# drowe67/radae

Measured on AMD Instinct MI355X. Metric: vocoder-feature frames/sec (enc+chan+dec), model19, higher is better.
Workload: dtype f32 I/O, 2xf16 (22-bit) MFMA operands, f32 accumulate (refine: f64 MFMA)

## Files before the change

radae_amd/csrc/rade_rx.hip:

```cpp
#include "rade_devutil.h"
typedef unsigned u32x2 __attribute__((ext_vector_type(2)));

#define DQ_XB 96
#define DQ_HB 16
#define DQ_PEND_MAX 64
#ifndef DQ_GIS
#define DQ_GIS 292
#endif
__device__ __forceinline__ int dq_xoff(int t, int col) { return (t + 1) * (DQ_XB * 8) + ((((col >> 3) ^ (t & 15)) << 3) | (col & 7)); }
__device__ __forceinline__ int dq_hoff(int t, int col) { return t * (DQ_HB * 8) + ((((col >> 3) ^ (t & 15)) << 3) | (col & 7)); }
__device__ __forceinline__ void dq_split(float v, _Float16 &hi, _Float16 &lo) { const float x = 256.0f * v; hi = (_Float16)x; lo = (_Float16)(x - (float)hi); }

enum { DQ_OUT_X = 0, DQ_OUT_GI = 1, DQ_OUT_GLOBAL = 2 };
struct DqGemm {
    const unsigned short *wa; int nct;
    const float *bias; int N;
    const float *wscale;
    int from_hb;
    int ktap;
    int ks0, nks;
    int init_gi;
    int out, ocol, act;
    float *gout; int gstride;
};
// ... 160 lines not shown
            if (act == 2) {
                const f16x4 hh = *(const lds_f16x4 *)(hbh + dq_hoff(tt, n)), hl = *(const lds_f16x4 *)(hbl + dq_hoff(tt, n));
#pragma unroll
                for (int r = 0; r < 4; r++) v[r] = clamp1(((float)hh[r] + (float)hl[r]) * 0x1p-8f * gate_sigmoid(v[r]));
            } else {
#pragma unroll
                for (int r = 0; r < 4; r++) v[r] = clamp1(gate_tanh(v[r]));
            }
            f16x4 oh, ol;
#pragma unroll
            for (int r = 0; r < 4; r++) { _Float16 a, b; dq_split(v[r], a, b); oh[r] = a; ol[r] = b; }
            *(lds_f16x4 *)(xh + dq_xoff(tt, ocol + n)) = oh; *(lds_f16x4 *)(xl + dq_xoff(tt, ocol + n)) = ol;
        }
    }
}
template <int NT>
__device__ __forceinline__ void dq2_gemm_tiles(DecShared2 *sh, const DqGemm g, int ct, int Tb, unsigned rstmask, int sync_first)
{
    if (uni_ptr(g.wscale) != nullptr) dq2_gemm_tiles_<NT, true>(sh, g, ct, Tb, rstmask, sync_first);
    else dq2_gemm_tiles_<NT, false>(sh, g, ct, Tb, rstmask, sync_first);
}

__device__ void dq2_dense1(DecShared2 *sh, const float *z, const rd_lin w, int Tb)
{
    constexpr int NKB = RD_LATENT / 8;
    const int lane = threadIdx.x & 63, nt = threadIdx.x >> 6, half = lane >> 5;
    if (nt >= 3) return;
    const float *wp = w.wp + ((size_t)nt * 64 + lane) * 4;
    const size_t wstep = (size_t)3 * 256;
    const int col = nt * 32 + (lane & 31);
    const float bias = w.bias[col];
    const int t = min(lane & 31, Tb - 1);
    const float *p1 = z + (size_t)t * RD_LATENT + 4 * half;
    f32x4 av[NKB], bv[NKB];
#pragma unroll
    for (int kb = 0; kb < NKB; kb++) { av[kb] = *(const f32x4 *)(p1 + kb * 8); bv[kb] = *(const f32x4 *)(wp + kb * wstep); }
    f32x16 acc;
#pragma unroll
    for (int j = 0; j < 16; j++) acc[j] = 0.0f;
#pragma unroll
    for (int kb = 0; kb < NKB; kb++)
#pragma unroll
        for (int s = 0; s < 4; s++) acc = __builtin_amdgcn_mfma_f32_32x32x2f32(av[kb][s], bv[kb][s], acc, 0, 0, 0);
#pragma unroll
    for (int j = 0; j < 16; j++) {
        const int tt = (j & 3) + 8 * (j >> 2) + 4 * half;
        if (tt >= Tb) continue;
        _Float16 a, b; dq_split(clamp1(gate_tanh(acc[j] + bias)), a, b);
        sh->xh[0][dq_xoff(tt, col)] = a; sh->xl[0][dq_xoff(tt, col)] = b;
    }
}

__device__ __forceinline__ f32x2 fma2(f32x2 a, f32x2 b, f32x2 c) { return (f32x2){ fmaf(a[0], b[0], c[0]), fmaf(a[1], b[1], c[1]) }; }
__device__ void dq2_scan(DecShared2 *sh, const float *Whh, const float *bhh, float *hstate, int Tb, unsigned rstmask)
{
    constexpr int H = 96, KP = H / 2;
    const int tid = rx_tid();
    const bool on = tid < 2 * H;
    const int j = on ? tid >> 1 : 0, p = tid & 1;
    f32x2 wr[KP / 2], wz[KP / 2], wn[KP / 2];
    {
        const float *w0 = Whh + (size_t)j * H + p * KP;
#pragma unroll
        for (int k = 0; k < KP; k += 4) {
            const f32x4 v0 = *(const f32x4 *)(w0 + k), v1 = *(const f32x4 *)(w0 + (size_t)H * H + k), v2 = *(const f32x4 *)(w0 + (size_t)2 * H * H + k);
#pragma unroll
            for (int u = 0; u < 2; u++) {
                wr[k / 2 + u] = (f32x2){ v0[2 * u], v0[2 * u + 1] }; wz[k / 2 + u] = (f32x2){ v1[2 * u], v1[2 * u + 1] }; wn[k / 2 + u] = (f32x2){ v2[2 * u], v2[2 * u + 1] };
            }
        }
    }
    const float br = bhh[j], bz = bhh[H + j], bn = bhh[2 * H + j];
    float hj = hstate[j];
    __syncthreads();
    if (on && p == 0) sh->hs[0][j] = hj;
    const float *gi = &sh->gi[0][0] + j;
    float g0r = gi[0], g0z = gi[H], g0n = gi[2 * H];
    __syncthreads();
    int cur = 0;
    for (int t = 0; t < Tb; t++) {
        if ((rstmask >> t) & 1u) {
            hj = 0.0f;
            __syncthreads();
            if (on && p == 0) sh->hs[cur][j] = 0.0f;
            __syncthreads();
        }
        const float *gn_ = gi + (size_t)min(t + 1, Tb - 1) * DQ_GIS;
        const float g1r = gn_[0], g1z = gn_[H], g1n = gn_[2 * H];
        f32x2 ar = { 0.0f, 0.0f }, az = { 0.0f, 0.0f }, an = { 0.0f, 0.0f }, ar2 = { 0.0f, 0.0f }, az2 = { 0.0f, 0.0f }, an2 = { 0.0f, 0.0f };
        const float *hp = sh->hs[cur] + p * KP;
#pragma unroll
        for (int k = 0; k < KP; k += 8) {
            const f32x4 hv = *(const f32x4 *)(hp + k), hw = *(const f32x4 *)(hp + k + 4);
            const f32x2 h0 = { hv[0], hv[1] }, h1 = { hv[2], hv[3] }, h2 = { hw[0], hw[1] }, h3 = { hw[2], hw[3] };
            ar = fma2(wr[k / 2], h0, ar); az = fma2(wz[k / 2], h0, az); an = fma2(wn[k / 2], h0, an);
            ar2 = fma2(wr[k / 2 + 1], h1, ar2); az2 = fma2(wz[k / 2 + 1], h1, az2); an2 = fma2(wn[k / 2 + 1], h1, an2);
            ar = fma2(wr[k / 2 + 2], h2, ar); az = fma2(wz[k / 2 + 2], h2, az); an = fma2(wn[k / 2 + 2], h2, an);
            ar2 = fma2(wr[k / 2 + 3], h3, ar2); az2 = fma2(wz[k / 2 + 3], h3, az2); an2 = fma2(wn[k / 2 + 3], h3, an2);
        }
        ar += ar2; az += az2; an += an2;
        float sr = ar[0] + ar[1], sz = az[0] + az[1], sn = an[0] + an[1];
        sr += quad_dpp<QUAD_XOR1>(sr); sz += quad_dpp<QUAD_XOR1>(sz); sn += quad_dpp<QUAD_XOR1>(sn);
        const float r = gate_sigmoid((sr + br) + g0r);
        const float z = gate_sigmoid((sz + bz) + g0z);
        const float n = gate_tanh(g0n + (sn + bn) * r);
        hj = (hj - n) * z + n;
        if (on && p == 0) {
            sh->hs[cur ^ 1][j] = hj;
            _Float16 a, b; dq_split(clamp1(hj), a, b);
            sh->hbh[0][dq_hoff(t, j)] = a; sh->hbl[0][dq_hoff(t, j)] = b;
        }
        g0r = g1r; g0z = g1z; g0n = g1n;
        cur ^= 1;
        if (t + 1 < Tb) __syncthreads();
    }
    if (on && p == 0) hstate[j] = hj;
}

template <int NB>
__device__ __forceinline__ void dq2_scan_mfma_body(DecShared2 *sh, const unsigned short *whq, const float *whs, const float *bhh, float *hstate, int Tb, unsigned rstmask, int ub0)
{
    constexpr int H = 96;
    const int tid = rx_tid(), lane = tid & 63, c = lane & 15, g = lane >> 4, cs = c & 3, par = c & 1;
    const int blk = NB == 2 ? (c >> 3) & 1 : 0;
    typedef const __attribute__((address_space(1))) f16x8 glb_f16x8_t;
    f16x8 A[NB][3][3];
    float sc[3], bb[3];
    const bool finl = (c & 4) == 0 && (NB == 2 || c < 4);
    const int ju = 16 * (ub0 + blk) + 4 * g + cs;
#pragma unroll
    for (int k = 0; k < NB; k++)
#pragma unroll
        for (int gate = 0; gate < 3; gate++)
#pragma unroll
            for (int ks = 0; ks < 3; ks++) A[k][gate][ks] = *(glb_f16x8_t *)(whq + (((size_t)ks * 18 + gate * 6 + ub0 + k) * 64 + lane) * 8);
#pragma unroll
    for (int gate = 0; gate < 3; gate++) { sc[gate] = whs[gate * H + ju] * 0x1p-8f; bb[gate] = bhh[gate * H + ju]; }
    float hj = hstate[ju];
    __syncthreads();
    _Float16 (*hp)[2][H] = (_Float16 (*)[2][H])&sh->hs[0][0];
    if (finl) { _Float16 a, b; dq_split(hj, a, b); hp[0][0][ju] = a; hp[0][1][ju] = b; }
    const float *gi = &sh->gi[0][0];
    float g0[3];
#pragma unroll
    for (int gate = 0; gate < 3; gate++) g0[gate] = gi[gate * H + ju];
    __syncthreads();
    int cur = 0;
    for (int t = 0; t < Tb; t++) {
        if ((rstmask >> t) & 1u) {
            __syncthreads();
            hj = 0.0f; if (finl) { hp[cur][0][ju] = (_Float16)0.0f; hp[cur][1][ju] = (_Float16)0.0f; }
            __syncthreads();
        }
        const float *gn_ = gi + (size_t)min(t + 1, Tb - 1) * DQ_GIS;
        float g1[3];
#pragma unroll
        for (int gate = 0; gate < 3; gate++) g1[gate] = gn_[gate * H + ju];
        f16x8 bq[3];
#pragma unroll
        for (int ks = 0; ks < 3; ks++) bq[ks] = *(const f16x8 *)&hp[cur][par][32 * ks + 8 * g];
        __builtin_amdgcn_sched_barrier(0);
        f32x4 acc[NB][3];
#pragma unroll
        for (int k = 0; k < NB; k++)
#pragma unroll
            for (int gate = 0; gate < 3; gate++) acc[k][gate] = (f32x4){ 0.0f, 0.0f, 0.0f, 0.0f };
#pragma unroll
        for (int ks = 0; ks < 3; ks++)
#pragma unroll
            for (int k = 0; k < NB; k++)
#pragma unroll
                for (int gate = 0; gate < 3; gate++) acc[k][gate] = __builtin_amdgcn_mfma_f32_16x16x32_f16(A[k][gate][ks], bq[ks], acc[k][gate], 0, 0, 0);
        float s3[3];
#pragma unroll
        for (int gate = 0; gate < 3; gate++) {
            float sr[4];
#pragma unroll
            for (int r = 0; r < 4; r++) {
                const float v = NB == 2 ? (blk ? acc[NB - 1][gate][r] : acc[0][gate][r]) : acc[0][gate][r];
                sr[r] = v + quad_dpp<QUAD_XOR1>(v); asm volatile("" : "+v"(sr[r]));
            }
            const float s01 = (cs & 1) ? sr[1] : sr[0], s23 = (cs & 1) ? sr[3] : sr[2];
            s3[gate] = (cs & 2) ? s23 : s01;
        }
        {
            const float r = gate_sigmoid((s3[0] * sc[0] + bb[0]) + g0[0]);
            const float z = gate_sigmoid((s3[1] * sc[1] + bb[1]) + g0[1]);
            const float n = gate_tanh(g0[2] + (s3[2] * sc[2] + bb[2]) * r);
            hj = (hj - n) * z + n;
        }
        if (finl) {
            _Float16 a, b; dq_split(hj, a, b);
            hp[cur ^ 1][0][ju] = a; hp[cur ^ 1][1][ju] = b;
            dq_split(clamp1(hj), a, b);
            sh->hbh[0][dq_hoff(t, ju)] = a; sh->hbl[0][dq_hoff(t, ju)] = b;
        }
#pragma unroll
        for (int gate = 0; gate < 3; gate++) g0[gate] = g1[gate];
        cur ^= 1;
        if (t + 1 < Tb) __syncthreads();
    }
    if (finl) hstate[ju] = hj;
}
__device__ void dq2_scan_mfma(DecShared2 *sh, const unsigned short *whq, const float *whs, const float *bhh, float *hstate, int Tb, unsigned rstmask)
{
    const int wave = rx2_wave();
    if (wave < 2) dq2_scan_mfma_body<2>(sh, whq, whs, bhh, hstate, Tb, rstmask, 2 * wave);
    else dq2_scan_mfma_body<1>(sh, whq, whs, bhh, hstate, Tb, rstmask, 2 + wave);
}

__device__ void dq2_layers(DecShared2 *sh, const rd_decs_args &a, int b, const float *z, float *out, int Tb, unsigned rstmask, int census_noscan)
{
    const int tid = rx_tid(), wave = tid >> 6;
    PH2_T0();
    {
        const unsigned *hist = (const unsigned *)(a.x + (size_t)b * a.x_sb - RD_DEC_W);
        constexpr int NH_ = (RD_DEC_W + NT2 - 1) / NT2;
        unsigned hu[NH_];
#pragma unroll
        for (int q = 0; q < NH_; q++) hu[q] = hist[min(tid + q * NT2, RD_DEC_W - 1)];
#pragma unroll
        for (int q = 0; q < NH_; q++) {
            const int c = tid + q * NT2; const unsigned u = hu[q];
            if (c < RD_DEC_W) { sh->xh[0][dq_xoff(-1, c)] = __builtin_bit_cast(_Float16, (unsigned short)(u & 0xffffu)); sh->xl[0][dq_xoff(-1, c)] = __builtin_bit_cast(_Float16, (unsigned short)(u >> 16)); }
        }
        for (int c = tid; c < DQ_XB * 8; c += NT2) { sh->xh[DQ2_ROWS + 1][c] = (_Float16)0.0f; sh->xl[DQ2_ROWS + 1][c] = (_Float16)0.0f; }
    }
    dq2_dense1(sh, z, a.dense1, Tb);
    DqGemm g;
    const int ct18 = wave < 2 ? 5 * wave : 10 + 4 * (wave - 2);
    g = (DqGemm){ a.gin[0].wa16, 18, a.gin[0].bias, 288, a.gin[0].wscale, 0, 0, 0, 3, 0, DQ_OUT_GI, 0, 0, nullptr, 0 };
    if (wave < 2) dq2_gemm_tiles<5>(sh, g, ct18, Tb, rstmask, 1); else dq2_gemm_tiles<4>(sh, g, ct18, Tb, rstmask, 1);
    PH2(20);
#pragma unroll 1
    for (int l = 0; l < 5; l++) {
        const int in = 96 + 128 * l, cin = in + 96;
        if (census_noscan) __syncthreads();
        else if (a.whq[l]) dq2_scan_mfma(sh, a.whq[l], a.whs[l], a.bhh[l], a.h[l] + (size_t)b * 96, Tb, rstmask);
        else dq2_scan(sh, a.whh[l], a.bhh[l], a.h[l] + (size_t)b * 96, Tb, rstmask);
        PH2(21);
        g = (DqGemm){ a.glu[l].wa16, 6, nullptr, 96, a.glu[l].wscale, 1, 0, 0, 3, 0, DQ_OUT_X, in, 2, nullptr, 0 };
        if (wave < 2) dq2_gemm_tiles<2>(sh, g, 2 * wave, Tb, rstmask, 1); else dq2_gemm_tiles<1>(sh, g, 2 + wave, Tb, rstmask, 1);
        PH2(22);
        const DqGemm gc = (DqGemm){ a.conv[l].wa16, 2, a.conv[l].bias, 32, a.conv[l].wscale, 0, cin / 32, 0, 2 * cin / 32, 0, DQ_OUT_X, cin, 1, nullptr, 0 };
        const bool last = l == 4;
        const rd_lin &nx = last ? a.output : a.gin[l + 1];
        const int nct = last ? 6 : 18;
        const DqGemm gm = (DqGemm){ nx.wa16, nct, nx.bias, last ? a.out_w : 288, nx.wscale, 0, 0, 0, cin / 32, 0, DQ_OUT_GI, 0, 0, nullptr, 0 };
        if (wave < 2) {
            dq2_gemm_tiles<1>(sh, gc, wave, Tb, rstmask, 1);
            if (!last) dq2_gemm_tiles<3>(sh, gm, 3 * wave, Tb, rstmask, 0);
        } else if (last) dq2_gemm_tiles<3>(sh, gm, 3 * (wave - 2), Tb, rstmask, 1);
        else {
            dq2_gemm_tiles<3>(sh, gm, 6 + 6 * (wave - 2), Tb, rstmask, 1);
            dq2_gemm_tiles<3>(sh, gm, 9 + 6 * (wave - 2), Tb, rstmask, 0);
        }
        PH2(23);
        const DqGemm gf = (DqGemm){ nx.wa16, nct, nullptr, last ? a.out_w : 288, nx.wscale, 0, 0, cin / 32, 1, 1, last ? DQ_OUT_GLOBAL : DQ_OUT_GI, 0, 0, out, a.out_w };
        if (last) { if (wave >= 2) dq2_gemm_tiles<3>(sh, gf, 3 * (wave - 2), Tb, rstmask, 1); else __syncthreads(); }
        else if (wave < 2) dq2_gemm_tiles<5>(sh, gf, ct18, Tb, rstmask, 1);
        else dq2_gemm_tiles<4>(sh, gf, ct18, Tb, rstmask, 1);
        PH2(24);
    }
    __syncthreads();
    {
        unsigned *hist = (unsigned *)(a.x + (size_t)b * a.x_sb - RD_DEC_W);
        for (int c = tid; c < RD_DEC_W; c += NT2)
            hist[c] = (unsigned)__builtin_bit_cast(unsigned short, sh->xh[0][dq_xoff(Tb - 1, c)]) | ((unsigned)__builtin_bit_cast(unsigned short, sh->xl[0][dq_xoff(Tb - 1, c)]) << 16);
    }
    __syncthreads();
}

struct RxShared2 {
    RxScalars S;
    double2 rq[4], rzc, rph[24], rrot[24]; double ral[24];
    int rows48[48];
    double redd[(NW2 + 1) * 10];
    float redf[16]; int redi[16]; int redj[16];
    double corrp[NW2][8];
    union {
      struct {
        float2 rxb[RD_RXBUF];
        float rowsum1[RD_NMF], rowsum2[RD_NMF];
        union {
          struct {
            __attribute__((aligned(16))) float2 xm[1408];
            double2 pd[RD_M], pendd[RD_M];
            float2 sym[6][RD_NC]; float2 rp[2][RD_NC];
            float eqP[RD_NC]; float2 eqPmat[RD_NC][2][3], eqrot[RD_NC]; float eq_pg, eq_snrc1, eq_snrc2, eq_pad;
            float2 cisA[2][18], cisB[2][64];
            union {
              struct {
                u32x2 rxhl[RD_RXBUF];
                double rmom[2][2][64][4];
                double mtot[2][16][16];
              };
              struct {
                double2 rtw[80], rrot80[80], rt80[80];
                float2 dtr[2 * 80 * 16];
              };
            };
          };
          struct {
            __attribute__((aligned(16))) _Float16 sA[2][2 * 2 * 2 * 64 * 8];
            __attribute__((aligned(16))) _Float16 sA2[5 * 2 * 64 * 8];
            unsigned srxh[RD_RXBUF], srxl[RD_RXBUF];
          };
        };
      };
      __attribute__((aligned(16))) unsigned char dec_raw[sizeof(DecShared2)];
    };
};
static_assert(sizeof(RxShared2) <= 80 * 1024, "two k_rx_sync2 workgroups must fit the 160 KiB LDS of a CU");

__device__ void block_argmax2(RxShared2 *sh, float &v, int &k0, int &k1)
{
    const int tid = rx_tid(), lane = tid & 63, wave = tid >> 6;
#define ARGMAX_STEP(CTRL) do { const float ov = quad_dpp<CTRL>(v); const int o0 = quad_dpp_i<CTRL>(k0), o1 = quad_dpp_i<CTRL>(k1); \
        if (ov > v || (ov == v && (o0 < k0 || (o0 == k0 && o1 < k1)))) { v = ov; k0 = o0; k1 = o1; } } while (0)
    ARGMAX_STEP(QUAD_XOR1); ARGMAX_STEP(QUAD_XOR2); ARGMAX_STEP(ROW_ROR4); ARGMAX_STEP(ROW_ROR8);
#undef ARGMAX_STEP
    {
        float bv = __int_as_float(__builtin_amdgcn_readlane(__float_as_int(v), 0)); int b0 = __builtin_amdgcn_readlane(k0, 0), b1 = __builtin_amdgcn_readlane(k1, 0);
#pragma unroll
        for (int r = 1; r < 4; r++) {
            const float ov = __int_as_float(__builtin_amdgcn_readlane(__float_as_int(v), 16 * r)); const int o0 = __builtin_amdgcn_readlane(k0, 16 * r), o1 = __builtin_amdgcn_readlane(k1, 16 * r);
            if (ov > bv || (ov == bv && (o0 < b0 || (o0 == b0 && o1 < b1)))) { bv = ov; b0 = o0; b1 = o1; }
        }
        v = bv; k0 = b0; k1 = b1;
    }
    if (lane == 0) { sh->redf[1 + wave] = v; sh->redi[1 + wave] = k0; sh->redj[1 + wave] = k1; }
    __syncthreads();
    float bv = sh->redf[1]; int b0 = sh->redi[1], b1 = sh->redj[1];
#pragma unroll
    for (int w = 1; w < NW2; w++) {
        const float ov = sh->redf[1 + w]; const int o0 = sh->redi[1 + w], o1 = sh->redj[1 + w];
        if (ov > bv || (ov == bv && (o0 < b0 || (o0 == b0 && o1 < b1)))) { bv = ov; b0 = o0; b1 = o1; }
    }
    v = bv; k0 = b0; k1 = b1;
}
template <int NV>
__device__ void block_sum_multi2(RxShared2 *sh, double (&v)[NV])
{
    const int tid = rx_tid(), lane = tid & 63, wave = tid >> 6;
#pragma unroll
    for (int k = 0; k < NV; k++) v[k] = wave_sum_f64(v[k]);
    if (lane == 0) {
#pragma unroll
        for (int k = 0; k < NV; k++) sh->redd[wave * NV + k] = v[k];
    }
    __syncthreads();
#pragma unroll
    for (int k = 0; k < NV; k++) {
        double t = 0.0;
#pragma unroll
        for (int w = 0; w < NW2; w++) t += sh->redd[w * NV + k];
        v[k] = t;
    }
}
__device__ float sigma_r_from_rowsums2(RxShared2 *sh)
{
    double v[2] = { 0.0, 0.0 };
    for (int t = rx_tid(); t < RD_NMF; t += NT2) { v[0] += (double)sh->rowsum1[t]; v[1] += (double)sh->rowsum2[t]; }
    block_sum_multi2<2>(sh, v);
    return sigma_r_from_sums(v[0], v[1]);
}


struct MomPlanes { f16x8 h, m, l; };
__device__ __forceinline__ MomPlanes mom_split(const f32x4 a0, const f32x4 a1)
{
    MomPlanes p;
#pragma unroll
    for (int j = 0; j < 8; j++) {
        const float v = 0x1p-7f * (j < 4 ? a0[j & 3] : a1[j & 3]);
        const _Float16 h = (_Float16)v; const float r1 = v - (float)h;
        const _Float16 m = (_Float16)r1; const float r2 = r1 - (float)m;
        p.h[j] = h; p.m[j] = m; p.l[j] = (_Float16)r2;
    }
    return p;
}
__device__ __forceinline__ f32x4 mom_expand(const f16x8 ah, const f16x8 al, const MomPlanes &p)
{
    f32x4 c = { 0.0f, 0.0f, 0.0f, 0.0f };
    c = __builtin_amdgcn_mfma_f32_16x16x32_f16(ah, p.l, c, 0, 0, 0);
    c = __builtin_amdgcn_mfma_f32_16x16x32_f16(al, p.m, c, 0, 0, 0);
    c = __builtin_amdgcn_mfma_f32_16x16x32_f16(al, p.h, c, 0, 0, 0);
    c = __builtin_amdgcn_mfma_f32_16x16x32_f16(ah, p.m, c, 0, 0, 0);
    c = __builtin_amdgcn_mfma_f32_16x16x32_f16(ah, p.h, c, 0, 0, 0);
    return c;
}
__device__ __forceinline__ void rx2_detect_q(RxShared2 *sh, const unsigned short *corrq16_, const unsigned short *corra16_, float *cache_, int cached, int oldb, int newb,
                                             float rx_unsc_, float &best, int &bt, int &bfi)
{
    constexpr int RT = 5, NTF = 5, TPW = 15;
    static_assert(TPW * NW2 * 16 == RD_NMF && TPW % RT == 0, "timing tiles per wavefront");
    const int tid = rx_tid(), wave = rx2_wave(), lane = tid & 63, i = lane & 15, g = lane >> 4;
    const float rx_unsc = rx_unsc_ * 0x1p-3f;
    const __amdgpu_buffer_rsrc_t qrs = __builtin_amdgcn_make_buffer_rsrc((void *)uni_ptr(corrq16_), 0, 2 * 10 * 2048, 0x00020000);
    const int vo = tid * 16;
    u32x4 stg[2];
    auto stage_load = [&](int sb) {
        stg[0] = __builtin_amdgcn_raw_buffer_load_b128(qrs, vo, sb * 4096, 0); stg[1] = __builtin_amdgcn_raw_buffer_load_b128(qrs, vo, sb * 4096 + 10 * 2048, 0);
    };
    auto stage_store = [&](int buf) { _Float16 *d = &sh->sA[buf][tid * 8]; *(u32x4 *)d = stg[0]; *(u32x4 *)(d + 256 * 8) = stg[1]; };
    PH2_T0();
    {
        const __amdgpu_buffer_rsrc_t ars = __builtin_amdgcn_make_buffer_rsrc((void *)uni_ptr(corra16_), 0, 5 * 2048, 0x00020000);
        const u32x4 t0 = __builtin_amdgcn_raw_buffer_load_b128(ars, vo, 0, 0), t1 = __builtin_amdgcn_raw_buffer_load_b128(ars, vo, 4096, 0);
        u32x4 t2 = { 0u, 0u, 0u, 0u };
        if (wave < 2) t2 = __builtin_amdgcn_raw_buffer_load_b128(ars, vo, 8192, 0);
        stage_load(0);
        _Float16 *d = &sh->sA2[tid * 8];
        *(u32x4 *)d = t0; *(u32x4 *)(d + 256 * 8) = t1;
        if (wave < 2) *(u32x4 *)(d + 512 * 8) = t2;
        stage_store(0);
    }
    float lbest = best; int lkey = 0x7fffffff;
    int pb = 0;
    __syncthreads();
    PH2(15);
#pragma unroll 1
    for (int pass = cached ? 1 : 0; pass < 2; pass++) {
        const unsigned *ph = sh->srxh + pass * RD_NMF + i + 4 * g, *pl = sh->srxl + pass * RD_NMF + i + 4 * g;
        const __amdgpu_buffer_rsrc_t drs = __builtin_amdgcn_make_buffer_rsrc((void *)uni_ptr(cache_ + (size_t)(pass ? newb : oldb) * RD_NFC * RD_NMF), 0, RD_NFC * RD_NMF * 4, 0x00020000);
        const __amdgpu_buffer_rsrc_t prs = __builtin_amdgcn_make_buffer_rsrc((void *)uni_ptr(cache_ + (size_t)oldb * RD_NFC * RD_NMF), 0, RD_NFC * RD_NMF * 4, 0x00020000);
        float *rowsum = pass ? sh->rowsum2 : sh->rowsum1;
#pragma unroll 1
        for (int grp = 0; grp < TPW / RT; grp++) {
            const int T0 = wave * TPW + grp * RT;
            f32x4 acc1[RT][2];
#pragma unroll
            for (int rt = 0; rt < RT; rt++) { acc1[rt][0] = (f32x4){ 0.0f, 0.0f, 0.0f, 0.0f }; acc1[rt][1] = (f32x4){ 0.0f, 0.0f, 0.0f, 0.0f }; }
            u32x4 wh[RT + 1], wl[RT + 1];
#pragma unroll
            for (int rt = 0; rt < RT; rt++)
#pragma unroll
                for (int j = 0; j < 4; j++) { wh[rt][j] = ph[16 * (T0 + rt) + j]; wl[rt][j] = pl[16 * (T0 + rt) + j]; }
#pragma unroll
            for (int sb = 0; sb < 5; sb++) {
                stage_load(sb == 4 ? 0 : sb + 1);
#pragma unroll
                for (int ds = 0; ds < 2; ds++) {
                    const int sidx = 2 * sb + ds;
                    if (sidx < 9) {
#pragma unroll
                        for (int j = 0; j < 4; j++) { wh[(RT + sidx) % (RT + 1)][j] = ph[16 * (T0 + RT + sidx) + j]; wl[(RT + sidx) % (RT + 1)][j] = pl[16 * (T0 + RT + sidx) + j]; }
                    }
                    const _Float16 *Ab = &sh->sA[pb][lane * 8];
                    const f16x8 a0h = *(const f16x8 *)(Ab + ((0 * 2 + ds) * 2 + 0) * 512), a0l = *(const f16x8 *)(Ab + ((0 * 2 + ds) * 2 + 1) * 512);
                    const f16x8 a1h = *(const f16x8 *)(Ab + ((1 * 2 + ds) * 2 + 0) * 512), a1l = *(const f16x8 *)(Ab + ((1 * 2 + ds) * 2 + 1) * 512);
                    __builtin_amdgcn_sched_barrier(0);
#define WSL(rt) (((rt) + sidx) % (RT + 1))
#pragma unroll
                    for (int rt = 0; rt < RT; rt++) acc1[rt][0] = __builtin_amdgcn_mfma_f32_16x16x32_f16(a0l, __builtin_bit_cast(f16x8, wh[WSL(rt)]), acc1[rt][0], 0, 0, 0);
#pragma unroll
                    for (int rt = 0; rt < RT; rt++) acc1[rt][1] = __builtin_amdgcn_mfma_f32_16x16x32_f16(a1l, __builtin_bit_cast(f16x8, wh[WSL(rt)]), acc1[rt][1], 0, 0, 0);
#pragma unroll
                    for (int rt = 0; rt < RT; rt++) acc1[rt][0] = __builtin_amdgcn_mfma_f32_16x16x32_f16(a0h, __builtin_bit_cast(f16x8, wl[WSL(rt)]), acc1[rt][0], 0, 0, 0);
#pragma unroll
                    for (int rt = 0; rt < RT; rt++) acc1[rt][1] = __builtin_amdgcn_mfma_f32_16x16x32_f16(a1h, __builtin_bit_cast(f16x8, wl[WSL(rt)]), acc1[rt][1], 0, 0, 0);
#pragma unroll
                    for (int rt = 0; rt < RT; rt++) acc1[rt][0] = __builtin_amdgcn_mfma_f32_16x16x32_f16(a0h, __builtin_bit_cast(f16x8, wh[WSL(rt)]), acc1[rt][0], 0, 0, 0);
#pragma unroll
                    for (int rt = 0; rt < RT; rt++) acc1[rt][1] = __builtin_amdgcn_mfma_f32_16x16x32_f16(a1h, __builtin_bit_cast(f16x8, wh[WSL(rt)]), acc1[rt][1], 0, 0, 0);
#undef WSL
                    __builtin_amdgcn_sched_barrier(0);
                }
                stage_store(pb ^ 1);
                pb ^= 1;
                __syncthreads();
            }
            PH2(16);
            f16x8 A2h[NTF], A2l[NTF];
#pragma unroll
            for (int q = 0; q < NTF; q++) { A2h[q] = *(const f16x8 *)&sh->sA2[((q * 2) * 64 + lane) * 8]; A2l[q] = *(const f16x8 *)&sh->sA2[((q * 2 + 1) * 64 + lane) * 8]; }
            const int gb = (wave * (TPW / RT) + grp) * RT * 2560;
            float pv[2][2 * NTF];
            auto pv_load = [&](int slot, int rt) {
                const u32x4 v0 = __builtin_amdgcn_raw_buffer_load_b128(prs, lane * 16, gb + rt * 2560, 0), v1 = __builtin_amdgcn_raw_buffer_load_b128(prs, lane * 16, gb + rt * 2560 + 1024, 0);
                const u32x2 v2 = __builtin_amdgcn_raw_buffer_load_b64(prs, lane * 8, gb + rt * 2560 + 2048, 0);
#pragma unroll
                for (int k = 0; k < 4; k++) { pv[slot][k] = __uint_as_float(v0[k]); pv[slot][4 + k] = __uint_as_float(v1[k]); }
                pv[slot][8] = __uint_as_float(v2[0]); pv[slot][9] = __uint_as_float(v2[1]);
            };
            if (pass) pv_load(0, 0);
            const int tb = 16 * T0 + i;
#pragma unroll
            for (int rt = 0; rt < RT; rt++) {
                if (pass && rt + 1 < RT) pv_load((rt + 1) & 1, rt + 1);
                const MomPlanes mp = mom_split(acc1[rt][0], acc1[rt][1]);
                float dd[2 * NTF], rs = 0.0f;
#pragma unroll
                for (int q = 0; q < NTF; q++) {
                    const f32x4 c = mom_expand(A2h[q], A2l[q], mp);
                    const float d0 = rx_unsc * __builtin_amdgcn_sqrtf(fmaf(c[0], c[0], c[1] * c[1])), d1 = rx_unsc * __builtin_amdgcn_sqrtf(fmaf(c[2], c[2], c[3] * c[3]));
                    rs += d0; rs += d1;
                    dd[2 * q] = d0; dd[2 * q + 1] = d1;
                }
                {
                    const auto p16 = __builtin_amdgcn_permlane16_swap(__float_as_uint(rs), __float_as_uint(rs), false, false);
                    rs = __uint_as_float(p16[0]) + __uint_as_float(p16[1]);
                    const auto p32 = __builtin_amdgcn_permlane32_swap(__float_as_uint(rs), __float_as_uint(rs), false, false);
                    rs = __uint_as_float(p32[0]) + __uint_as_float(p32[1]);
                }
                __builtin_amdgcn_raw_buffer_store_b128((u32x4){ __float_as_uint(dd[0]), __float_as_uint(dd[1]), __float_as_uint(dd[2]), __float_as_uint(dd[3]) }, drs, lane * 16, gb + rt * 2560, 0);
                __builtin_amdgcn_raw_buffer_store_b128((u32x4){ __float_as_uint(dd[4]), __float_as_uint(dd[5]), __float_as_uint(dd[6]), __float_as_uint(dd[7]) }, drs, lane * 16, gb + rt * 2560 + 1024, 0);
                __builtin_amdgcn_raw_buffer_store_b64((u32x2){ __float_as_uint(dd[8]), __float_as_uint(dd[9]) }, drs, lane * 8, gb + rt * 2560 + 2048, 0);
                const int t = tb + 16 * rt;
                if (pass) {
#pragma unroll
                    for (int q = 0; q < NTF; q++) {
                        const int k0 = (t << 6) | (8 * q + 2 * g);
                        const float s0 = pv[rt & 1][2 * q] + dd[2 * q], s1 = pv[rt & 1][2 * q + 1] + dd[2 * q + 1];
                        const bool c0 = s0 > lbest; lbest = c0 ? s0 : lbest; lkey = c0 ? k0 : lkey;
                        const bool c1 = s1 > lbest; lbest = c1 ? s1 : lbest; lkey = c1 ? k0 + 1 : lkey;
                    }
                }
                if (g == 0) rowsum[t] = rs;
            }
            PH2(17);
        }
        __syncthreads();
        PH2(18);
    }
    best = lbest; bt = lkey >> 6; bfi = lkey & 63;
}

__device__ __forceinline__ f64x4 refine2_tile(const RxShared2 *sh, int mt, int frame, int s0, int ns, int nf, int nt, int lane)
{
    const int i = lane & 15, kk = lane >> 4, c = kk & 1, n0 = kk >> 1;
    const int row = 16 * mt + i, fi = row >> 1, cp = row & 1;
    const bool rv = fi < nf;
    const double2 z1 = sh->rtw[rv ? fi : 0];
    double2 cur = s0 ? sh->rt80[rv ? fi : 0] : make_double2(1.0, 0.0);
    if (n0) cur = make_double2(cur.x * z1.x - cur.y * z1.y, cur.x * z1.y + cur.y * z1.x);
    const double c2r = z1.x * z1.x - z1.y * z1.y, c2i = 2.0 * z1.x * z1.y;
    const double2 prv = make_double2(cur.x * c2r + cur.y * c2i, cur.y * c2r - cur.x * c2i);
    double xc = cp == c ? cur.x : (cp == 0 ? -cur.y : cur.y), xp = cp == c ? prv.x : (cp == 0 ? -prv.y : prv.y);
    if (!rv) { xc = 0.0; xp = 0.0; }
    const double k2 = 2.0 * c2r;
    const double *xw = (const double *)&sh->xm[0] + 4 * (frame * 176 + (i < nt ? i : 0) + 2 * s0 + n0) + 2 * c;
    const double2 *pp = &sh->pd[2 * s0 + n0];
    f64x4 acc0 = { 0.0, 0.0, 0.0, 0.0 }, acc1 = acc0;
    double2 pn[4]; double a1[4], a2[4];
#pragma unroll
    for (int u = 0; u < 4; u++) { pn[u] = pp[2 * u]; a1[u] = xw[8 * u]; a2[u] = xw[8 * u + 1]; }
#pragma unroll 1
    for (int s = 0; s < ns; s += 4) {
        double b[4];
#pragma unroll
        for (int u = 0; u < 4; u++) b[u] = pn[u].x * a1[u];
#pragma unroll
        for (int u = 0; u < 4; u++) b[u] = fma(pn[u].y, a2[u], b[u]);
        __builtin_amdgcn_sched_barrier(0);
        const int sn = s + 4 < ns ? s + 4 : s;
#pragma unroll
        for (int u = 0; u < 4; u++) { pn[u] = pp[2 * (sn + u)]; a1[u] = xw[8 * (sn + u)]; a2[u] = xw[8 * (sn + u) + 1]; }
        __builtin_amdgcn_sched_barrier(0);
        const double x1 = fma(k2, xc, -xp), x2 = fma(k2, x1, -xc), x3 = fma(k2, x2, -x1);
        acc0 = __builtin_amdgcn_mfma_f64_16x16x4f64(xc, b[0], acc0, 0, 0, 0);
        acc1 = __builtin_amdgcn_mfma_f64_16x16x4f64(x1, b[1], acc1, 0, 0, 0);
        acc0 = __builtin_amdgcn_mfma_f64_16x16x4f64(x2, b[2], acc0, 0, 0, 0);
        acc1 = __builtin_amdgcn_mfma_f64_16x16x4f64(x3, b[3], acc1, 0, 0, 0);
        xp = x3; xc = fma(k2, x3, -x2);
        __builtin_amdgcn_sched_barrier(0);
    }
    return acc0 + acc1;
}
__device__ __forceinline__ void refine2_tables(RxShared2 *sh, int k, double fstart, double fstop, double fstep)
{
    const int nf = (int)ceil((fstop - fstart) / fstep);
    const double delta = (fstart + fstep) - fstart;
    if (k < 0 || k >= 3 * nf) return;
    const int which = k / nf, fi = k - which * nf;
    const double w = 2.0 * PI_D * dgrid_nc(fstart, fi, delta) / 8000.0;
    const double arg = which == 0 ? -w : (which == 1 ? -w * RD_NMF : -w * 80.0);
    double sn, cs; sincos(arg, &sn, &cs);
    double2 *dstp = which == 0 ? sh->rtw : (which == 1 ? sh->rrot80 : sh->rt80);
    dstp[fi] = make_double2(cs, sn);
}
__device__ __forceinline__ void refine2_tables_sync(RxShared2 *sh, int k, double fstart, double fstop, double fstep)
{
    const int nf = (int)ceil((fstop - fstart) / fstep);
    const double delta = (fstart + fstep) - fstart;
    const double wc = 0.5 * (2.0 * PI_D * fstart / 8000.0 + 2.0 * PI_D * dgrid_nc(fstart, nf - 1, delta) / 8000.0);
    if (k < 0 || k > 52) return;
    const int kf = k < 24 ? k : k - 24;
    if (k < 48 && kf >= nf) return;
    const double w = 2.0 * PI_D * dgrid_nc(fstart, kf, delta) / 8000.0, dw = w - wc;
    const double arg = k < 24 ? -w * RD_NMF : (k < 48 ? -dw * 79.5 : (k < 52 ? -wc * 40.0 * (k - 48) : -wc));
    double sn, cs; sincos(arg, &sn, &cs);
    const double2 v = make_double2(cs, sn);
    if (k < 24) sh->rrot[k] = v;
    else if (k < 48) { sh->rph[kf] = v; sh->ral[kf] = dw * 80.0; }
    else if (k < 52) sh->rq[k - 48] = v;
    else sh->rzc = v;
}
__device__ __forceinline__ void refine2_moments(const RxShared2 *sh, const double *vmg, int frame, int q, int nt, int lane, f64x4 &acc0, f64x4 &acc1)
{
    const int i = lane & 15, kk = lane >> 4, c = kk & 1, n0 = kk >> 1;
    const int m = i >> 1, cp = i & 1, s0 = 20 * q;
    const double2 z1 = sh->rzc;
    double2 cur = sh->rq[q];
    if (n0) cur = make_double2(cur.x * z1.x - cur.y * z1.y, cur.x * z1.y + cur.y * z1.x);
    const double c2r = z1.x * z1.x - z1.y * z1.y, c2i = 2.0 * z1.x * z1.y;
    const double2 prv = make_double2(cur.x * c2r + cur.y * c2i, cur.y * c2r - cur.x * c2i);
    double xc = cp == c ? cur.x : (cp == 0 ? -cur.y : cur.y), xp = cp == c ? prv.x : (cp == 0 ? -prv.y : prv.y);
    const double k2 = 2.0 * c2r;
    const double *xw = (const double *)&sh->xm[0] + 4 * (frame * 176 + (i < nt ? i : 0) + 2 * s0 + n0) + 2 * c;
    const double2 *pp = &sh->pd[2 * s0 + n0];
    const __attribute__((address_space(1))) double *vp = (const __attribute__((address_space(1))) double *)vmg + m * RD_M + 2 * s0 + n0;
    double vall[20];
#pragma unroll
    for (int u = 0; u < 20; u++) vall[u] = vp[2 * u];
    double2 pn[4]; double a1[4], a2[4];
#pragma unroll
    for (int u = 0; u < 4; u++) { pn[u] = pp[2 * u]; a1[u] = xw[8 * u]; a2[u] = xw[8 * u + 1]; }
#pragma unroll
    for (int s = 0; s < 20; s += 4) {
        double b[4];
#pragma unroll
        for (int u = 0; u < 4; u++) b[u] = pn[u].x * a1[u];
#pragma unroll
        for (int u = 0; u < 4; u++) b[u] = fma(pn[u].y, a2[u], b[u]);
        __builtin_amdgcn_sched_barrier(0);
        const int sn = s + 4 < 20 ? s + 4 : s;
#pragma unroll
        for (int u = 0; u < 4; u++) { pn[u] = pp[2 * (sn + u)]; a1[u] = xw[8 * (sn + u)]; a2[u] = xw[8 * (sn + u) + 1]; }
        __builtin_amdgcn_sched_barrier(0);
        const double x1 = fma(k2, xc, -xp), x2 = fma(k2, x1, -xc), x3 = fma(k2, x2, -x1);
        acc0 = __builtin_amdgcn_mfma_f64_16x16x4f64(xc * vall[s], b[0], acc0, 0, 0, 0);
        acc1 = __builtin_amdgcn_mfma_f64_16x16x4f64(x1 * vall[s + 1], b[1], acc1, 0, 0, 0);
        acc0 = __builtin_amdgcn_mfma_f64_16x16x4f64(x2 * vall[s + 2], b[2], acc0, 0, 0, 0);
        acc1 = __builtin_amdgcn_mfma_f64_16x16x4f64(x3 * vall[s + 3], b[3], acc1, 0, 0, 0);
        xp = x3; xc = fma(k2, x3, -x2);
        __builtin_amdgcn_sched_barrier(0);
    }
}

__device__ void rx2_refine(RxShared2 *sh, const double *vmg, int *tmax, double *fmax, int t0, int nt, double fstart, double fstop, double fstep, bool in_sync)
{
    const int tid = rx_tid(), lane = tid & 63, wave = tid >> 6;
    const int nf = (int)ceil((fstop - fstart) / fstep);
    const double delta = (fstart + fstep) - fstart;
    const int ntasks = ((2 * nf + 15) >> 4) * 2;
    const int i = lane & 15, kk = lane >> 4;
    PH2_T0();
    if (!in_sync) refine2_tables(sh, tid, fstart, fstop, fstep);
    for (int j = tid; j < 2 * 176; j += NT2) {
        const int frame = j / 176, k = j - frame * 176;
        const float2 x = sh->rxb[min(t0 + frame * RD_NMF + k, RD_RXBUF - 1)];
        double *d = (double *)&sh->xm[0] + 4 * j;
        d[0] = (double)x.x; d[1] = (double)x.y; d[2] = (double)x.y; d[3] = -(double)x.x;
    }
    __syncthreads();
    PH2(27);
    float best = -1.0f; int bf = 0x7fffffff, bt = 0x7fffffff;
    if (in_sync) {
        {
            f64x4 a0 = { 0.0, 0.0, 0.0, 0.0 }, a1 = a0;
            refine2_moments(sh, vmg, wave & 1, 2 * (wave >> 1), nt, lane, a0, a1);
            refine2_moments(sh, vmg, wave & 1, 2 * (wave >> 1) + 1, nt, lane, a0, a1);
            const f64x4 part = a0 + a1;
#pragma unroll
            for (int r = 0; r < 4; r++) sh->rmom[wave >> 1][wave & 1][lane][r] = part[r];
        }
        __syncthreads();
        PH2(28);
        for (int o = tid; o < 2 * 64 * 4; o += NT2) {
            const int frame = o >> 8, l = (o >> 2) & 63, r = o & 3;
            sh->mtot[frame][(l >> 4) + 4 * r][l & 15] = sh->rmom[0][frame][l][r] + sh->rmom[1][frame][l][r];
        }
        __syncthreads();
        PH2(29);
        for (int o = tid; o < nf * 16; o += NT2) {
            const int fo = o >> 4, t = o & 15;
            if (t >= nt) continue;
            const double al = sh->ral[fo];
            const double2 ph = sh->rph[fo], rt = sh->rrot[fo];
            float2 d12[2];
#pragma unroll
            for (int frame = 0; frame < 2; frame++) {
                double re = 0.0, im = 0.0, cm = 1.0;
#pragma unroll
                for (int mq = 0; mq < 8; mq++) {
                    const double mr = sh->mtot[frame][2 * mq][t], mi = sh->mtot[frame][2 * mq + 1][t];
                    if ((mq & 3) == 0) { re = fma(cm, mr, re); im = fma(cm, mi, im); }
                    else if ((mq & 3) == 1) { re = fma(cm, mi, re); im = fma(-cm, mr, im); }
                    else if ((mq & 3) == 2) { re = fma(-cm, mr, re); im = fma(-cm, mi, im); }
                    else { re = fma(-cm, mi, re); im = fma(cm, mr, im); }
                    cm = cm * al * (1.0 / (double)(mq + 1));
                }
                double xr = re * ph.x - im * ph.y, xi = re * ph.y + im * ph.x;
                if (frame == 1) { const double tr = xr * rt.x - xi * rt.y; xi = xr * rt.y + xi * rt.x; xr = tr; }
                d12[frame] = make_float2((float)xr, (float)xi);
            }
            const float v = hypotf(d12[0].x + d12[1].x, d12[0].y + d12[1].y);
            if (v > best || (v == best && (fo < bf || (fo == bf && t < bt)))) { best = v; bf = fo; bt = t; }
        }
    } else {
        auto finish = [&](const f64x4 &acc, int mt, int frame) {
#pragma unroll
            for (int r = 0; r < 4; r++) {
                const double mine = acc[r], other = __shfl_xor(mine, 16);
                if ((kk & 1) == 0) {
                    const int fo = 8 * mt + (kk >> 1) + 2 * r;
                    double re = mine, im = other;
                    if (frame == 1 && fo < nf) {
                        const double2 rt = sh->rrot80[fo];
                        const double tr = re * rt.x - im * rt.y; im = re * rt.y + im * rt.x; re = tr;
                    }
                    if (fo < nf && i < nt) sh->dtr[(frame * nf + fo) * 16 + i] = make_float2((float)re, (float)im);
                }
            }
        };
        for (int task = wave; task < ntasks; task += NW2) finish(refine2_tile(sh, task >> 1, task & 1, 0, 80, nf, nt, lane), task >> 1, task & 1);
        __syncthreads();
        for (int task = tid; task < nf * nt; task += NT2) {
            const int fi = task / nt, ti = task - fi * nt;
            const float2 a = sh->dtr[fi * 16 + ti], b = sh->dtr[(nf + fi) * 16 + ti];
            const float v = hypotf(a.x + b.x, a.y + b.y);
            if (v > best || (v == best && (fi < bf || (fi == bf && ti < bt)))) { best = v; bf = fi; bt = ti; }
        }
    }
    PH2(30);
    block_argmax2(sh, best, bf, bt);
    PH2(31);
    if (best > 0.0f) { *tmax = t0 + bt; *fmax = dgrid_nc(fstart, bf, delta); }
}

__device__ __forceinline__ void rx2_load_rxbuf(RxShared2 *sh, const rd_rx_stream *st, int tid)
{
    constexpr int NB_ = (RD_RXBUF + NT2 - 1) / NT2, NR_ = (RD_NMF + NT2 - 1) / NT2;
    float2 v[NB_]; float r1[NR_], r2[NR_];
#pragma unroll
    for (int q = 0; q < NB_; q++) { const int i = min(tid + q * NT2, RD_RXBUF - 1); v[q] = make_float2(st->rx_buf[i][0], st->rx_buf[i][1]); }
#pragma unroll
    for (int q = 0; q < NR_; q++) { const int i = min(tid + q * NT2, RD_NMF - 1); r1[q] = st->rowsum1[i]; r2[q] = st->rowsum2[i]; }
#pragma unroll
    for (int q = 0; q < NB_; q++) { const int i = tid + q * NT2; if (i < RD_RXBUF) sh->rxb[i] = v[q]; }
#pragma unroll
    for (int q = 0; q < NR_; q++) { const int i = tid + q * NT2; if (i < RD_NMF) { sh->rowsum1[i] = r1[q]; sh->rowsum2[i] = r2[q]; } }
}

__device__ __forceinline__ void rx2_decode_pending(RxShared2 *sh, const rd_sync_args &a, int b)
{
    RxScalars *S = &sh->S;
    DecShared2 *ds = (DecShared2 *)&sh->dec_raw[0];
    rd_rx_round *rnd = a.round + b;
    rd_rx_stream *st = a.st + b;
    const int tid = rx_tid();
    const int Tb = S->n_rows;
    PH2_T0();
    for (int i = tid; i < RD_RXBUF; i += NT2) { st->rx_buf[i][0] = sh->rxb[i].x; st->rx_buf[i][1] = sh->rxb[i].y; }
    for (int i = tid; i < RD_NMF; i += NT2) { st->rowsum1[i] = sh->rowsum1[i]; st->rowsum2[i] = sh->rowsum2[i]; }
    __syncthreads();
    PH2(19);
    for (int i = tid; i < Tb; i += NT2) ds->rst[i] = rnd->row_reset[i];
    if (tid == 0) S->lds_sync = 0;
    __syncthreads();
    for (int c0 = 0; c0 < Tb; c0 += DQ2_ROWS) {
        const int n = min(DQ2_ROWS, Tb - c0);
        unsigned rstmask = 0u;
        for (int t = 0; t < n; t++) rstmask |= ds->rst[c0 + t] ? (1u << t) : 0u;
        if (!CENSUS(1)) dq2_layers(ds, a.dec, b, a.dec.z + (size_t)b * a.dec.z_sb + (size_t)c0 * RD_LATENT, a.dec.out + (size_t)b * a.dec.out_sb + (size_t)c0 * a.dec.out_w, n, rstmask, CENSUS(2));
    }
    const float *f84 = a.dec.out + (size_t)b * a.dec.out_sb;
    for (int r = tid; r < Tb; r += NT2) ds->err[r] = f84[r * 84 + 20] > 0.0f ? 1 : 0;
    float *out = a.features_out + (size_t)b * a.feat_stride + (size_t)S->out_base * RD_FEAT_MF;
    for (int i0 = tid; i0 < (Tb / 3) * RD_FEAT_MF; i0 += 4 * NT2) {
        float v[4];
#pragma unroll
        for (int q = 0; q < 4; q++) {
            const int i = min(i0 + q * NT2, (Tb / 3) * RD_FEAT_MF - 1), fr = i / 36, j = i - fr * 36;
            const int row = fr >> 2, sub = fr & 3;
            v[q] = f84[row * 84 + sub * 21 + min(j, 19)];
            if (j >= 20) v[q] = 0.0f;
        }
#pragma unroll
        for (int q = 0; q < 4; q++) { const int i = i0 + q * NT2; if (i < (Tb / 3) * RD_FEAT_MF) out[i] = v[q]; }
    }
    __syncthreads();
    if (a.trace) {
        for (int c = S->batch_call0 + tid; c < S->n_calls; c += NT2) {
            const int idx = rnd->call_trace_idx[c];
            if (idx >= a.trace_cap) continue;
            int e = 0;
            for (int r = rnd->call_row_lo[c]; r < rnd->call_row_hi[c]; r++) e += ds->err[r];
            a.trace[(size_t)b * a.trace_cap + idx].uw_errors += e;
        }
    }
    if (tid == 0) {
        int add = 0;
        for (int r = S->uw_from_row; r < Tb; r++) add += ds->err[r];
        S->uw_errors += add;
        S->out_base += Tb / 3; S->n_rows = 0; S->uw_from_row = 0; S->pending_valid = 0; S->batch_call0 = S->n_calls; S->need_decode = 0;
    }
    __syncthreads();
    PH2_RESTART();
    rx2_load_rxbuf(sh, st, tid);
    __syncthreads();
    PH2(19);
}

__device__ __forceinline__ void rx2_bypass_pending(RxShared2 *sh, const rd_sync_args &a, int b)
{
    RxScalars *S = &sh->S;
    const int tid = rx_tid();
    const int Tb = S->n_rows;
    const float *z = a.dec.z + (size_t)b * a.dec.z_sb;
    float *out = a.features_out + (size_t)b * a.feat_stride + (size_t)S->out_base * RD_ZMF;
    for (int i = tid; i < Tb * RD_LATENT; i += NT2) out[i] = z[i];
    __syncthreads();
    if (tid == 0) { S->out_base += Tb / 3; S->n_rows = 0; S->uw_from_row = 0; S->pending_valid = 0; S->batch_call0 = S->n_calls; S->need_decode = 0; }
    __syncthreads();
}

typedef __attribute__((address_space(3))) const u32x2 lds_cu32x2;
template <int NRT, int DA, class Pre, class Side>
__device__ __forceinline__ void check2_rows_q(RxShared2 *sh, const unsigned short *corrq16_, const unsigned short *corra16_, int frame, int rt0, int lane, float rx_unsc_, Pre pre, Side side)
{
// ... 853 lines not shown
```

Baseline: 83.36 million.

## Stream detection A operands from global into registers instead of LDS double buffer

The correlation A-operand slices now load directly from global memory into registers per wave, prefetched two steps ahead, instead of being staged cooperatively through an LDS double buffer with a workgroup barrier after each stage. This removes five __syncthreads per group and the sA LDS buffer. The previous-pass values are now prefetched earlier, overlapped with the final MFMA step, and the next group's first A slices are prefetched during the epilogue. In exchange every wave issues its own redundant global loads and register pressure rises (AL/AH arrays, pv[5][10]), which may reduce occupancy or cause spills.

```diff
diff --git a/radae_amd/csrc/rade_rx.hip b/radae_amd/csrc/rade_rx.hip
--- a/radae_amd/csrc/rade_rx.hip
+++ b/radae_amd/csrc/rade_rx.hip
@@ -486,7 +486,6 @@
             };
           };
           struct {
-            __attribute__((aligned(16))) _Float16 sA[2][2 * 2 * 2 * 64 * 8];
             __attribute__((aligned(16))) _Float16 sA2[5 * 2 * 64 * 8];
             unsigned srxh[RD_RXBUF], srxl[RD_RXBUF];
           };
@@ -578,30 +577,33 @@
                                              float rx_unsc_, float &best, int &bt, int &bfi)
 {
     constexpr int RT = 5, NTF = 5, TPW = 15;
+    constexpr int AREQ = 3;
     static_assert(TPW * NW2 * 16 == RD_NMF && TPW % RT == 0, "timing tiles per wavefront");
     const int tid = rx_tid(), wave = rx2_wave(), lane = tid & 63, i = lane & 15, g = lane >> 4;
     const float rx_unsc = rx_unsc_ * 0x1p-3f;
     const __amdgpu_buffer_rsrc_t qrs = __builtin_amdgcn_make_buffer_rsrc((void *)uni_ptr(corrq16_), 0, 2 * 10 * 2048, 0x00020000);
     const int vo = tid * 16;
-    u32x4 stg[2];
-    auto stage_load = [&](int sb) {
-        stg[0] = __builtin_amdgcn_raw_buffer_load_b128(qrs, vo, sb * 4096, 0); stg[1] = __builtin_amdgcn_raw_buffer_load_b128(qrs, vo, sb * 4096 + 10 * 2048, 0);
+    u32x4 nxL[2][2], nxH[2][2];
+    auto fetchL = [&](u32x4 (&d)[2], int s) {
+#pragma unroll
+        for (int u = 0; u < 2; u++) d[u] = __builtin_amdgcn_raw_buffer_load_b128(qrs, lane * 16, ((u * 10 + s) * 2 + 1) * 1024, 0);
     };
-    auto stage_store = [&](int buf) { _Float16 *d = &sh->sA[buf][tid * 8]; *(u32x4 *)d = stg[0]; *(u32x4 *)(d + 256 * 8) = stg[1]; };
+    auto fetchH = [&](u32x4 (&d)[2], int s) {
+#pragma unroll
+        for (int u = 0; u < 2; u++) d[u] = __builtin_amdgcn_raw_buffer_load_b128(qrs, lane * 16, ((u * 10 + s) * 2 + 0) * 1024, 0);
+    };
     PH2_T0();
     {
         const __amdgpu_buffer_rsrc_t ars = __builtin_amdgcn_make_buffer_rsrc((void *)uni_ptr(corra16_), 0, 5 * 2048, 0x00020000);
         const u32x4 t0 = __builtin_amdgcn_raw_buffer_load_b128(ars, vo, 0, 0), t1 = __builtin_amdgcn_raw_buffer_load_b128(ars, vo, 4096, 0);
         u32x4 t2 = { 0u, 0u, 0u, 0u };
         if (wave < 2) t2 = __builtin_amdgcn_raw_buffer_load_b128(ars, vo, 8192, 0);
-        stage_load(0);
+        fetchL(nxL[0], 0); fetchH(nxH[0], 0); fetchL(nxL[1], 1); fetchH(nxH[1], 1);
         _Float16 *d = &sh->sA2[tid * 8];
         *(u32x4 *)d = t0; *(u32x4 *)(d + 256 * 8) = t1;
         if (wave < 2) *(u32x4 *)(d + 512 * 8) = t2;
-        stage_store(0);
     }
     float lbest = best; int lkey = 0x7fffffff;
-    int pb = 0;
     __syncthreads();
     PH2(15);
 #pragma unroll 1
@@ -621,58 +623,56 @@
             for (int rt = 0; rt < RT; rt++)
 #pragma unroll
                 for (int j = 0; j < 4; j++) { wh[rt][j] = ph[16 * (T0 + rt) + j]; wl[rt][j] = pl[16 * (T0 + rt) + j]; }
-#pragma unroll
-            for (int sb = 0; sb < 5; sb++) {
-                stage_load(sb == 4 ? 0 : sb + 1);
-#pragma unroll
-                for (int ds = 0; ds < 2; ds++) {
-                    const int sidx = 2 * sb + ds;
-                    if (sidx < 9) {
-#pragma unroll
-                        for (int j = 0; j < 4; j++) { wh[(RT + sidx) % (RT + 1)][j] = ph[16 * (T0 + RT + sidx) + j]; wl[(RT + sidx) % (RT + 1)][j] = pl[16 * (T0 + RT + sidx) + j]; }
-                    }
-                    const _Float16 *Ab = &sh->sA[pb][lane * 8];
-                    const f16x8 a0h = *(const f16x8 *)(Ab + ((0 * 2 + ds) * 2 + 0) * 512), a0l = *(const f16x8 *)(Ab + ((0 * 2 + ds) * 2 + 1) * 512);
-                    const f16x8 a1h = *(const f16x8 *)(Ab + ((1 * 2 + ds) * 2 + 0) * 512), a1l = *(const f16x8 *)(Ab + ((1 * 2 + ds) * 2 + 1) * 512);
-                    __builtin_amdgcn_sched_barrier(0);
+            const int gb = (wave * (TPW / RT) + grp) * RT * 2560;
+            float pv[RT][2 * NTF];
+            auto pv_load = [&](int rt) {
+                const u32x4 v0 = __builtin_amdgcn_raw_buffer_load_b128(prs, lane * 16, gb + rt * 2560, 0), v1 = __builtin_amdgcn_raw_buffer_load_b128(prs, lane * 16, gb + rt * 2560 + 1024, 0);
+                const u32x2 v2 = __builtin_amdgcn_raw_buffer_load_b64(prs, lane * 8, gb + rt * 2560 + 2048, 0);
+#pragma unroll
+                for (int k = 0; k < 4; k++) { pv[rt][k] = __uint_as_float(v0[k]); pv[rt][4 + k] = __uint_as_float(v1[k]); }
+                pv[rt][8] = __uint_as_float(v2[0]); pv[rt][9] = __uint_as_float(v2[1]);
+            };
+            u32x4 AL[10][2], AH[10][2];
+#pragma unroll
+            for (int u = 0; u < 2; u++) { AL[0][u] = nxL[0][u]; AH[0][u] = nxH[0][u]; AL[1][u] = nxL[1][u]; AH[1][u] = nxH[1][u]; }
+#pragma unroll
+            for (int sidx = 0; sidx < 10; sidx++) {
+                if (sidx < 9) {
+#pragma unroll
+                    for (int j = 0; j < 4; j++) { wh[(RT + sidx) % (RT + 1)][j] = ph[16 * (T0 + RT + sidx) + j]; wl[(RT + sidx) % (RT + 1)][j] = pl[16 * (T0 + RT + sidx) + j]; }
+                }
+                if (sidx + 2 < 10) fetchL(AL[sidx + 2], sidx + 2);
+                const f16x8 a0h = __builtin_bit_cast(f16x8, AH[sidx][0]), a0l = __builtin_bit_cast(f16x8, AL[sidx][0]);
+                const f16x8 a1h = __builtin_bit_cast(f16x8, AH[sidx][1]), a1l = __builtin_bit_cast(f16x8, AL[sidx][1]);
+                __builtin_amdgcn_sched_barrier(0);
 #define WSL(rt) (((rt) + sidx) % (RT + 1))
 #pragma unroll
-                    for (int rt = 0; rt < RT; rt++) acc1[rt][0] = __builtin_amdgcn_mfma_f32_16x16x32_f16(a0l, __builtin_bit_cast(f16x8, wh[WSL(rt)]), acc1[rt][0], 0, 0, 0);
-#pragma unroll
-                    for (int rt = 0; rt < RT; rt++) acc1[rt][1] = __builtin_amdgcn_mfma_f32_16x16x32_f16(a1l, __builtin_bit_cast(f16x8, wh[WSL(rt)]), acc1[rt][1], 0, 0, 0);
-#pragma unroll
-                    for (int rt = 0; rt < RT; rt++) acc1[rt][0] = __builtin_amdgcn_mfma_f32_16x16x32_f16(a0h, __builtin_bit_cast(f16x8, wl[WSL(rt)]), acc1[rt][0], 0, 0, 0);
-#pragma unroll
-                    for (int rt = 0; rt < RT; rt++) acc1[rt][1] = __builtin_amdgcn_mfma_f32_16x16x32_f16(a1h, __builtin_bit_cast(f16x8, wl[WSL(rt)]), acc1[rt][1], 0, 0, 0);
-#pragma unroll
-                    for (int rt = 0; rt < RT; rt++) acc1[rt][0] = __builtin_amdgcn_mfma_f32_16x16x32_f16(a0h, __builtin_bit_cast(f16x8, wh[WSL(rt)]), acc1[rt][0], 0, 0, 0);
-#pragma unroll
-                    for (int rt = 0; rt < RT; rt++) acc1[rt][1] = __builtin_amdgcn_mfma_f32_16x16x32_f16(a1h, __builtin_bit_cast(f16x8, wh[WSL(rt)]), acc1[rt][1], 0, 0, 0);
+                for (int rt = 0; rt < RT; rt++) acc1[rt][0] = __builtin_amdgcn_mfma_f32_16x16x32_f16(a0l, __builtin_bit_cast(f16x8, wh[WSL(rt)]), acc1[rt][0], 0, 0, 0);
+#pragma unroll
+                for (int rt = 0; rt < RT; rt++) acc1[rt][1] = __builtin_amdgcn_mfma_f32_16x16x32_f16(a1l, __builtin_bit_cast(f16x8, wh[WSL(rt)]), acc1[rt][1], 0, 0, 0);
+                __builtin_amdgcn_sched_barrier(0);
+                if (sidx + 2 < 10) fetchH(AH[sidx + 2], sidx + 2);
+                if (pass && sidx == 9) { pv_load(0); pv_load(1); }
+                __builtin_amdgcn_sched_barrier(0);
+#pragma unroll
+                for (int rt = 0; rt < RT; rt++) acc1[rt][0] = __builtin_amdgcn_mfma_f32_16x16x32_f16(a0h, __builtin_bit_cast(f16x8, wl[WSL(rt)]), acc1[rt][0], 0, 0, 0);
+#pragma unroll
+                for (int rt = 0; rt < RT; rt++) acc1[rt][1] = __builtin_amdgcn_mfma_f32_16x16x32_f16(a1h, __builtin_bit_cast(f16x8, wl[WSL(rt)]), acc1[rt][1], 0, 0, 0);
+#pragma unroll
+                for (int rt = 0; rt < RT; rt++) acc1[rt][0] = __builtin_amdgcn_mfma_f32_16x16x32_f16(a0h, __builtin_bit_cast(f16x8, wh[WSL(rt)]), acc1[rt][0], 0, 0, 0);
+#pragma unroll
+                for (int rt = 0; rt < RT; rt++) acc1[rt][1] = __builtin_amdgcn_mfma_f32_16x16x32_f16(a1h, __builtin_bit_cast(f16x8, wh[WSL(rt)]), acc1[rt][1], 0, 0, 0);
 #undef WSL
-                    __builtin_amdgcn_sched_barrier(0);
-                }
-                stage_store(pb ^ 1);
-                pb ^= 1;
-                __syncthreads();
+                __builtin_amdgcn_sched_barrier(0);
             }
             PH2(16);
             f16x8 A2h[NTF], A2l[NTF];
 #pragma unroll
             for (int q = 0; q < NTF; q++) { A2h[q] = *(const f16x8 *)&sh->sA2[((q * 2) * 64 + lane) * 8]; A2l[q] = *(const f16x8 *)&sh->sA2[((q * 2 + 1) * 64 + lane) * 8]; }
-            const int gb = (wave * (TPW / RT) + grp) * RT * 2560;
-            float pv[2][2 * NTF];
-            auto pv_load = [&](int slot, int rt) {
-                const u32x4 v0 = __builtin_amdgcn_raw_buffer_load_b128(prs, lane * 16, gb + rt * 2560, 0), v1 = __builtin_amdgcn_raw_buffer_load_b128(prs, lane * 16, gb + rt * 2560 + 1024, 0);
-                const u32x2 v2 = __builtin_amdgcn_raw_buffer_load_b64(prs, lane * 8, gb + rt * 2560 + 2048, 0);
-#pragma unroll
-                for (int k = 0; k < 4; k++) { pv[slot][k] = __uint_as_float(v0[k]); pv[slot][4 + k] = __uint_as_float(v1[k]); }
-                pv[slot][8] = __uint_as_float(v2[0]); pv[slot][9] = __uint_as_float(v2[1]);
-            };
-            if (pass) pv_load(0, 0);
             const int tb = 16 * T0 + i;
 #pragma unroll
             for (int rt = 0; rt < RT; rt++) {
-                if (pass && rt + 1 < RT) pv_load((rt + 1) & 1, rt + 1);
+                if (pass) { if (rt == 0) pv_load(2); if (rt + 3 < RT) pv_load(rt + 3); }
                 const MomPlanes mp = mom_split(acc1[rt][0], acc1[rt][1]);
                 float dd[2 * NTF], rs = 0.0f;
 #pragma unroll
@@ -692,16 +692,19 @@
                 __builtin_amdgcn_raw_buffer_store_b128((u32x4){ __float_as_uint(dd[4]), __float_as_uint(dd[5]), __float_as_uint(dd[6]), __float_as_uint(dd[7]) }, drs, lane * 16, gb + rt * 2560 + 1024, 0);
                 __builtin_amdgcn_raw_buffer_store_b64((u32x2){ __float_as_uint(dd[8]), __float_as_uint(dd[9]) }, drs, lane * 8, gb + rt * 2560 + 2048, 0);
                 const int t = tb + 16 * rt;
+                PH2(17);
                 if (pass) {
 #pragma unroll
                     for (int q = 0; q < NTF; q++) {
                         const int k0 = (t << 6) | (8 * q + 2 * g);
-                        const float s0 = pv[rt & 1][2 * q] + dd[2 * q], s1 = pv[rt & 1][2 * q + 1] + dd[2 * q + 1];
+                        const float s0 = pv[rt][2 * q] + dd[2 * q], s1 = pv[rt][2 * q + 1] + dd[2 * q + 1];
                         const bool c0 = s0 > lbest; lbest = c0 ? s0 : lbest; lkey = c0 ? k0 : lkey;
                         const bool c1 = s1 > lbest; lbest = c1 ? s1 : lbest; lkey = c1 ? k0 + 1 : lkey;
                     }
                 }
+                PH2(4);
                 if (g == 0) rowsum[t] = rs;
+                if (rt == AREQ) { fetchL(nxL[0], 0); fetchH(nxH[0], 0); fetchL(nxL[1], 1); fetchH(nxH[1], 1); }
             }
             PH2(17);
         }
```

Result: faster. 84.29 million, median of 6 (+1.1%).
